# SAP/nested-hashing-psi

Hardware: AMD Instinct MI355X
Metric: server PIE ciphertexts/sec (higher is better)
Workload: dtype u64

## Files before the change

include/piehip.h:

```cpp
#ifndef PIEHIP_H
#define PIEHIP_H

#include <stddef.h>
#include <stdint.h>

#ifdef __cplusplus
extern "C" {
#endif

#define PIEHIP_OK 0
#define PIEHIP_EINVAL (-1)
#define PIEHIP_ESTATE (-2)
#define PIEHIP_EHIP (-3)
#define PIEHIP_ENOMEM (-4)

typedef struct piehip_ctx *piehip_handle;

int piehip_version(void);
const char *piehip_last_error(void);

int piehip_default_moduli(uint32_t N, uint32_t L, uint64_t *q , uint64_t *p );

int piehip_create(piehip_handle *out, uint32_t N, uint32_t L, uint64_t t, const uint64_t *q, const uint64_t *p,
                  int device, void *stream);
// ... 74 lines not shown
int piehip_rccl_attach(piehip_handle h, void *nccl_comm, int nranks, int rank);
int piehip_rccl_destroy(piehip_handle h);
int piehip_rccl_bin_slice(uint32_t b_total, int nranks, int rank, uint32_t *bin_lo, uint32_t *bin_hi);
int piehip_rccl_broadcast(piehip_handle h, int root, void *d_buf, size_t bytes);
int piehip_rccl_broadcast_query(piehip_handle h, int root);
int piehip_gather_results(piehip_handle h, uint32_t b_total, int root, void *d_out);
int piehip_gather_results_host(piehip_handle h, uint32_t b_total, int root, uint64_t **results);
int piehip_rccl_wait(piehip_handle h, uint32_t timeout_ms);
int piehip_rccl_abort(piehip_handle h);
int piehip_rccl_agree(piehip_handle h, int ok, int *all_ok, uint32_t timeout_ms);

int piehip_ntt(piehip_handle h, uint64_t *limbs, uint32_t nlimbs, uint32_t mod_base, uint32_t mod_count, int inverse);
int piehip_eval_add(piehip_handle h, const uint64_t *x, const uint64_t *y, uint64_t *out);
int piehip_eval_mult_plain(piehip_handle h, const uint64_t *x, const uint64_t *pt, uint64_t *out);
int piehip_eval_mult(piehip_handle h, const uint64_t *x, const uint64_t *y, uint32_t nct, int relin, uint64_t *out);
int piehip_eval_automorph(piehip_handle h, const uint64_t *x, uint32_t g, const uint64_t *rk, uint64_t *out);
int piehip_encode(piehip_handle h, const int64_t *slots, uint32_t npt, uint32_t B, uint64_t *out);
int piehip_base_convert(piehip_handle h, int which, const uint64_t *in, uint32_t npoly, uint64_t *out);

int piehip_rotation_galois(piehip_handle h, int32_t index, uint32_t *g);
int piehip_load_rotation_keys(piehip_handle h, uint32_t nkeys, const int32_t *indices, const uint64_t *keys);
int piehip_fhepie_load_table(piehip_handle h, uint32_t npie, uint32_t K, uint32_t b, uint32_t E, const int64_t *slots,
                             const int64_t *masks);
int piehip_fhepie_set_index(piehip_handle h, const uint64_t *idx);
int piehip_fhepie_run(piehip_handle h);
int piehip_fhepie_get_results(piehip_handle h, uint64_t *out);

int piehip_client_keygen(piehip_handle h, uint64_t seed, uint64_t *sk);
int piehip_client_relin_keygen(piehip_handle h, const uint64_t *sk, uint64_t seed, uint64_t *evk);
int piehip_client_rot_keygen(piehip_handle h, const uint64_t *sk, int32_t index, uint64_t seed, uint64_t *rk);
int piehip_client_encrypt(piehip_handle h, const uint64_t *sk, const int64_t *slots, uint32_t nct, uint32_t B,
                          const uint64_t *seeds, uint64_t *out);
int piehip_client_decrypt(piehip_handle h, const uint64_t *sk, const uint64_t *ct, uint32_t nct, uint32_t B, int64_t *slots);

int piehip_expand_uniform(piehip_handle h, const uint8_t *seeds , uint32_t n, uint64_t *out );
int piehip_expand_uniform_device(piehip_handle h, const uint8_t *seeds , uint32_t n, void *d_out );
int piehip_stage_minus_seeded_q(piehip_handle h, uint32_t q, const uint64_t *c0 , const uint8_t *seed );
int piehip_stage_index_row_seeded_q(piehip_handle h, uint32_t q, uint32_t row, const uint64_t *c0 ,
                                    const uint8_t *seeds );
int piehip_stage_index_ct_seeded_q(piehip_handle h, uint32_t q, uint32_t row, uint32_t j, const uint64_t *c0 ,
                                   const uint8_t *seed );
int piehip_run_host_seeded_async(piehip_handle h, const uint64_t *c0idx, const uint8_t *idx_seeds, const uint64_t *c0minus,
                                 const uint8_t *minus_seeds, uint64_t *results);
int piehip_run_host_seeded(piehip_handle h, const uint64_t *c0idx, const uint8_t *idx_seeds, const uint64_t *c0minus,
                           const uint8_t *minus_seeds, uint64_t *results);
int piehip_load_relin_key_seeded(piehip_handle h, const uint64_t *evk0 , const uint8_t *seeds );
int piehip_load_relin_key_seeded_q(piehip_handle h, uint32_t q, const uint64_t *evk0, const uint8_t *seeds);
int piehip_client_encrypt_seeded(piehip_handle h, const uint64_t *sk, const int64_t *slots, uint32_t nct, uint32_t B,
                                 const uint64_t *noise_seeds , const uint8_t *a_seeds ,
                                 uint64_t *c0 );
int piehip_client_relin_keygen_seeded(piehip_handle h, const uint64_t *sk, uint64_t seed, const uint8_t *a_seeds ,
                                      uint64_t *evk0 );

#define PIEHIP_NKERNELS 13
enum {
    PIEHIP_K_STAGE_A = 0,
    PIEHIP_K_NTT_FWD = 1,
    PIEHIP_K_NTT_INV = 2,
    PIEHIP_K_EXPAND = 3,
    PIEHIP_K_TENSOR = 4,
    PIEHIP_K_SCALE = 5,
    PIEHIP_K_DIGITS = 6,
    PIEHIP_K_RELIN = 7,
    PIEHIP_K_MASK = 8,
    PIEHIP_K_ENCODE = 9,
    PIEHIP_K_AUTOMORPH = 10,
    PIEHIP_K_OTHER = 11,
    PIEHIP_K_EVENT_PAIR = 12
};
int piehip_bench_ntt(piehip_handle h, uint32_t nlimbs, uint32_t mod_count, int flags, uint32_t iters, double *ms_per_launch);
int piehip_set_profiling(piehip_handle h, int on);
#define PIEHIP_NKERNELS_V100 12
int piehip_profile_read_n(piehip_handle h, uint32_t n, uint32_t *launches , double *ms , double *alg_bytes );
int piehip_profile_read(piehip_handle h, uint32_t *launches , double *ms , double *alg_bytes );
const char *piehip_kernel_name(int k);

#ifdef __cplusplus
}
#endif
#endif
```

nested_hashing_psi_amd/_lib.py:

```python
import ctypes as C
import os

from .build import LIB_PATH

u64p = C.POINTER(C.c_uint64)
u8p = C.POINTER(C.c_uint8)
i64p = C.POINTER(C.c_int64)
u32p = C.POINTER(C.c_uint32)
i32p = C.POINTER(C.c_int32)
f64p = C.POINTER(C.c_double)

NKERNELS = 13

SYMBOLS = {
    "piehip_version": (C.c_int, []),
    "piehip_last_error": (C.c_char_p, []),
    "piehip_kernel_name": (C.c_char_p, [C.c_int]),
    "piehip_default_moduli": (C.c_int, [C.c_uint32, C.c_uint32, u64p, u64p]),
    "piehip_create": (C.c_int, [C.POINTER(C.c_void_p), C.c_uint32, C.c_uint32, C.c_uint64, u64p, u64p, C.c_int, C.c_void_p]),
    "piehip_destroy": (C.c_int, [C.c_void_p]),
    "piehip_get_moduli": (C.c_int, [C.c_void_p, u64p]),
    "piehip_get_root": (C.c_int, [C.c_void_p, C.c_uint32, u64p]),
    "piehip_get_twiddles": (C.c_int, [C.c_void_p, C.c_uint32, u64p, u64p]),
    "piehip_get_slot_positions": (C.c_int, [C.c_void_p, u32p]),
    "piehip_load_relin_key": (C.c_int, [C.c_void_p, u64p]),
    "piehip_load_db": (C.c_int, [C.c_void_p, C.c_uint32, C.c_uint32, C.c_uint32, u64p, u64p]),
    "piehip_load_db_slots": (C.c_int, [C.c_void_p, C.c_uint32, C.c_uint32, C.c_uint32, C.c_uint32, i64p, i64p]),
    "piehip_build_db": (C.c_int, [C.c_void_p, u64p, C.c_size_t] + [C.c_uint32] * 5 + [C.c_uint64] * 4),
    "piehip_load_db_table": (C.c_int, [C.c_void_p, u64p] + [C.c_uint32] * 5 + [C.c_uint64] * 2),
    "piehip_build_db_bins": (C.c_int, [C.c_void_p, u64p, C.c_size_t] + [C.c_uint32] * 5 + [C.c_uint64] * 4 + [C.c_uint32] * 2),
    "piehip_load_db_table_bins": (C.c_int, [C.c_void_p, u64p] + [C.c_uint32] * 5 + [C.c_uint64] * 2 + [C.c_uint32] * 2),
    "piehip_reserve": (C.c_int, [C.c_void_p, C.c_size_t] + [C.c_uint32] * 7),
    "piehip_get_hash_table": (C.c_int, [C.c_void_p, u64p]),
    "piehip_tabulation_hash": (C.c_int, [C.c_uint64, C.c_uint32, C.c_uint32, u64p, C.c_size_t, u64p]),
    "piehip_client_cuckoo_table": (C.c_int, [C.c_uint64, C.c_uint32, C.c_uint32, C.c_uint32, u64p, C.c_size_t, u64p]),
    "piehip_set_index": (C.c_int, [C.c_void_p, u64p]),
    "piehip_set_minus": (C.c_int, [C.c_void_p, u64p]),
    "piehip_set_index_device": (C.c_int, [C.c_void_p, C.c_void_p]),
    "piehip_set_minus_device": (C.c_int, [C.c_void_p, C.c_void_p]),
    "piehip_run": (C.c_int, [C.c_void_p]),
    "piehip_sync": (C.c_int, [C.c_void_p]),
    "piehip_join": (C.c_int, [C.c_void_p]),
    "piehip_run_into": (C.c_int, [C.c_void_p, C.c_void_p]),
    "piehip_run_host": (C.c_int, [C.c_void_p, u64p, u64p, u64p]),
    "piehip_run_host_async": (C.c_int, [C.c_void_p, u64p, u64p, u64p]),
    "piehip_run_host_wait": (C.c_int, [C.c_void_p]),
    "piehip_stage_minus": (C.c_int, [C.c_void_p, u64p]),
    "piehip_stage_index_row": (C.c_int, [C.c_void_p, C.c_uint32, u64p]),
    "piehip_run_staged": (C.c_int, [C.c_void_p, u64p]),
    "piehip_stage_minus_q": (C.c_int, [C.c_void_p, C.c_uint32, u64p]),
    "piehip_stage_index_row_q": (C.c_int, [C.c_void_p, C.c_uint32, C.c_uint32, u64p]),
    "piehip_stage_index_ct_q": (C.c_int, [C.c_void_p, C.c_uint32, C.c_uint32, C.c_uint32, u64p]),
    "piehip_stage_reset": (C.c_int, [C.c_void_p]),
    "piehip_host_buffers_q": (C.c_int, [C.c_void_p, C.c_uint32, C.POINTER(u64p), C.POINTER(u64p), C.POINTER(u64p)]),
    "piehip_load_relin_key_q": (C.c_int, [C.c_void_p, C.c_uint32, u64p]),
    "piehip_host_buffers": (C.c_int, [C.c_void_p, C.POINTER(u64p), C.POINTER(u64p), C.POINTER(u64p)]),
    "piehip_set_run_streams": (C.c_int, [C.c_void_p, C.c_uint32]),
    "piehip_set_graph": (C.c_int, [C.c_void_p, C.c_int]),
    "piehip_attach_database": (C.c_int, [C.c_void_p, C.c_void_p]),
    "piehip_set_query_batch": (C.c_int, [C.c_void_p, C.c_uint32]),
    "piehip_get_query_batch": (C.c_int, [C.c_void_p, u32p]),
    "piehip_set_index_q": (C.c_int, [C.c_void_p, C.c_uint32, u64p]),
    "piehip_set_minus_q": (C.c_int, [C.c_void_p, C.c_uint32, u64p]),
    "piehip_set_index_device_q": (C.c_int, [C.c_void_p, C.c_uint32, C.c_void_p]),
    "piehip_set_minus_device_q": (C.c_int, [C.c_void_p, C.c_uint32, C.c_void_p]),
# ... 78 lines not shown
```

nested_hashing_psi_amd/csrc/kernels.hpp:

```cpp
#pragma once
#include <hip/hip_runtime.h>

#include <atomic>
#include <vector>

#include "params.hpp"

namespace piehip {

struct PerDeviceOnce {
    std::atomic<unsigned long long> done{0};
    bool first_on_current_device()
    {
        int dev = 0;
        if (hipGetDevice(&dev) != hipSuccess || dev < 0 || dev > 63) return true;
        const unsigned long long bit = 1ULL << dev;
        return (done.fetch_or(bit) & bit) == 0;
    }
};

struct NttPlan {
    const u64 *tables;
    const u64 *twp;
    const u64 *twc;
    const u64 *twc_fold;
    const u64 *twk16 = nullptr;
    const u64 *twk16_fold = nullptr;
    const DevConsts *dc;
    u32 N, logN;
    u32 num_cus;
    u32 max_slots = 0;
    bool force_generic;
    u32 transform_cus() const
    {
        if (!max_slots) return num_cus;
        const u32 c = (max_slots + 1) / 2;
        return c < num_cus ? (c ? c : 1u) : num_cus;
    }
};

void build_twc_table(const u64 *nat_pairs, u32 logN, u32 s0, std::vector<u64> &out);
u32 ntt_fast_s0(u32 logN);
struct NttExtra {
    u64 *copy_out = nullptr;
    u32 copy_K = 1, copy_L = 1, copy_M = 1;
    u32 skip_L = 0, skip_M = 0;
    bool lazy_out = false;
    bool folded = false;
    bool x_lane_in = false;
};
void build_twk16_table(const u64 *nat_pairs, u32 s0, u32 slice_log, std::vector<u64> &out);
void ntt16_sigma_inverse_map(u32 logN, u32 s0, std::vector<u32> &map);
struct Ntt16Digits {
    const u64 *d2;
    size_t stride2;
    u64 *dig;
    u32 nb, L;
};
bool launch_ntt16(const NttPlan &pl, bool folded, u64 *data, u32 nlimbs, u32 mod_base, u32 mod_count, bool inverse, bool sigma,
                  hipStream_t st, const NttExtra *ex, const Ntt16Digits *dg = nullptr);
inline bool ntt16_applies(const NttPlan &pl, bool folded)
{
    return !pl.force_generic && pl.twp && (folded ? (pl.twk16_fold && (pl.logN == 14 || pl.logN == 15)) : (pl.twk16 && pl.logN == 13));
}
bool launch_ntt_fast(const u64 *twp, const u64 *twc, const DevConsts *dc, u32 N, u32 logN, u32 s0, u64 *data, u32 nlimbs, u32 mod_base,
                     u32 mod_count, bool inverse, bool sigma, u32 num_cus, hipStream_t st, const u64 *lift_src = nullptr,
                     u32 lift_L = 0, u32 sigma_split = 0, const NttExtra *ex = nullptr);
bool ntt_supports_extra(const NttPlan &pl, bool folded);
bool launch_ntt_digits(const NttPlan &pl, const u64 *d2, u64 *dig, u32 nb, u32 L, bool sigma, bool folded_layout,
                       hipStream_t st);
void ntt_sigma_inverse_map(u32 logN, u32 s0, std::vector<u32> &map);
void launch_ntt(const NttPlan &pl, u64 *data, u32 nlimbs, u32 mod_base, u32 mod_count, bool inverse, hipStream_t st,
                bool sigma = false, bool folded = false, const NttExtra *ex = nullptr);

struct StageAXOut {
    u64 *out = nullptr;
    u32 M = 0, logns = 0;
};
void launch_stage_a(const DevConsts *dc, u32 N, u32 L, u32 K, u32 b, u32 E, const u64 *idx, const u64 *minus,
                    const u64 *db, u64 *acc, hipStream_t st, bool small_moduli, u32 bstride = 0, u32 h0 = 0, u32 hn = 0, u32 nq = 1,
                    u32 q = 0, const StageAXOut *xo = nullptr);
static const u32 STAGE_A_MAX_QUERIES = 8;
struct StageAQueries {
    const u64 *idx[STAGE_A_MAX_QUERIES];
    const u64 *minus[STAGE_A_MAX_QUERIES];
};
void launch_stage_a_batch(const DevConsts *dc, u32 N, u32 L, u32 K, u32 b, u32 E, const StageAQueries &qs, u32 nq, const u64 *db,
                          u64 *acc, hipStream_t st, bool small_moduli, u32 bstride = 0, u32 h0 = 0, u32 hn = 0,
                          const StageAXOut *xo = nullptr);

void set_small_moduli(bool v);

void launch_expand_q_to_qp(const DevConsts *dc, u32 N, u32 L, const u64 *in, size_t in_stride_outer,
                           size_t in_stride_inner, u32 n_outer, u64 *out, u32 out_polys, u32 out_slot, hipStream_t st,
                           bool fold = false, bool skip_q = false);
void launch_scale_pq_expand(const DevConsts *dc, u32 N, u32 L, const u64 *in, size_t in_stride_outer,
                            size_t in_stride_inner, u32 n_outer, u64 *out, u32 out_polys, u32 out_slot, hipStream_t st,
                            bool fold = false);
void launch_expand_both(const DevConsts *dc, u32 N, u32 L, const u64 *x, size_t sx, const u64 *y, size_t sy, size_t si, u32 n_outer,
                        u64 *out, hipStream_t st, bool fold = false, bool skip_q = false);
void launch_tensor(const DevConsts *dc, u32 N, u32 M, const u64 *e, u64 *d, u32 nb, hipStream_t st);
void launch_scale_round(const DevConsts *dc, u32 N, u32 L, const u64 *d, u32 nb, u64 *out01, size_t stride01, u64 *out2,
                        size_t stride2, hipStream_t st, bool fold = false, bool fold_comp2 = false);
void launch_digits(const DevConsts *dc, u32 N, u32 L, const u64 *d2, size_t stride2, u32 nb, u64 *dig, hipStream_t st,
                   bool fold = false);
void launch_relin_mac(const DevConsts *dc, u32 N, u32 L, const u64 *d01, size_t stride01, const u64 *dig, const u64 *key,
                      const u64 *mask, u64 *out, u32 nb, hipStream_t st, const u32 *out_map = nullptr, size_t key_stride = 0,
                      u32 key_group = 1, u32 sigma_T = 0, u32 sigma_kp = 16, u32 mask_div = 1);
void launch_bcast_mul_plain(const DevConsts *dc, u32 N, u32 L, const u64 *x, size_t xs, u32 group, const u64 *pt, size_t ps_outer,
                            size_t ps_inner, u64 *out, u32 nct, hipStream_t st);
void launch_rot_prepare(const DevConsts *dc, u32 N, u32 L, const u64 *x, const u32 *maps, u32 map_group, bool acc, bool identity_first,
                        u64 *d01, u64 *d2, u32 nct, hipStream_t st);
void launch_sum_mul_plain(const DevConsts *dc, u32 N, u32 L, const u64 *x, u32 group, const u64 *pt, size_t pt_stride, u64 *out,
// ... 37 lines not shown
```

nested_hashing_psi_amd/csrc/kernels_ntt16.hip:

```cpp
#include "kernels.hpp"
#include "ntt16_kernel.h"

namespace piehip {

void build_twk16_table(const u64 *nat_pairs, u32 s0, u32 slice_log, std::vector<u64> &out)
{
    if (slice_log == 14)
        ntt16::build_twk_table_t<14>(nat_pairs, s0, out);
    else
        ntt16::build_twk_table_t<13>(nat_pairs, s0, out);
}

void ntt16_sigma_inverse_map(u32 logN, u32 s0, std::vector<u32> &map)
{
    const u32 N = 1u << logN, n = N >> s0;
    map.resize(N);
    for (u32 p = 0; p < N; p++) map[p] = (p / n) * n + ntt16::lane_to_std_t(p % n, n / 16);
}

template <u32 LOGNS>
static void launch_ntt16_t(const ntt16::Args &a, bool inverse, bool lift, u32 num_cus, hipStream_t st)
{
    typedef ntt16::Geo<LOGNS> G;
    constexpr size_t lds = (size_t)G::LDS_WORDS * sizeof(u64);
    static PerDeviceOnce attr[3];
    if (attr[inverse ? 1 : (lift ? 2 : 0)].first_on_current_device()) {
        if (inverse)
            (void)hipFuncSetAttribute((const void *)ntt16::ntt16_kernel_t<LOGNS, true>, hipFuncAttributeMaxDynamicSharedMemorySize, (int)lds);
        else if (lift)
            (void)hipFuncSetAttribute((const void *)ntt16::ntt16_kernel_t<LOGNS, false, true>, hipFuncAttributeMaxDynamicSharedMemorySize, (int)lds);
        else
            (void)hipFuncSetAttribute((const void *)ntt16::ntt16_kernel_t<LOGNS, false>, hipFuncAttributeMaxDynamicSharedMemorySize, (int)lds);
    }
    const u32 slots = (LOGNS == 13 ? 2u : 1u) * num_cus;
    const u32 grid = a.nitems < slots ? a.nitems : slots;
    if (inverse)
        hipLaunchKernelGGL((ntt16::ntt16_kernel_t<LOGNS, true>), dim3(grid), dim3(G::T), lds, st, a);
    else if (lift)
        hipLaunchKernelGGL((ntt16::ntt16_kernel_t<LOGNS, false, true>), dim3(grid), dim3(G::T), lds, st, a);
    else
        hipLaunchKernelGGL((ntt16::ntt16_kernel_t<LOGNS, false>), dim3(grid), dim3(G::T), lds, st, a);
}

bool launch_ntt16(const NttPlan &pl, bool folded, u64 *data, u32 nlimbs, u32 mod_base, u32 mod_count, bool inverse, bool sigma,
                  hipStream_t st, const NttExtra *ex, const Ntt16Digits *dg)
{
    const u64 *twk = folded ? pl.twk16_fold : pl.twk16;
    const u32 s0 = folded ? 1u : 0u;
    const u32 slice_log = pl.logN - s0;
    if (pl.force_generic || !twk || !pl.twp || (slice_log != 13 && slice_log != 14)) return false;
    if (!inverse && !sigma) return false;
    ntt16::Args a;
    a.data = data;
    a.twp = reinterpret_cast<const ntt16::u64x2 *>(pl.twp);
    a.twk = reinterpret_cast<const ntt16::u64x2 *>(twk);
    a.dc = pl.dc;
    a.N = pl.N;
    a.s0 = s0;
    a.nitems = nlimbs << s0;
    a.mod_base = mod_base;
    a.mod_count = mod_count;
    a.flags = 0;
    if (inverse && !sigma) a.flags |= ntt16::F_STD_IN;
    if (inverse && folded) a.flags |= ntt16::F_FOLDED;
    if (inverse && !sigma && ex && ex->copy_out && ex->x_lane_in) a.flags |= ntt16::F_X_LANE_IN;
    if (!inverse && ex && ex->lazy_out) a.flags |= ntt16::F_LAZY_OUT;
    a.skip_L = (ex && !inverse) ? ex->skip_L : 0;
    a.skip_M = ex ? ex->skip_M : 0;
    a.copy_out = (ex && inverse && !sigma) ? ex->copy_out : nullptr;
    a.copy_K = ex ? ex->copy_K : 1;
    a.copy_L = ex ? ex->copy_L : 1;
    a.copy_M = ex ? ex->copy_M : 1;
    a.lift_first = ~0u;
    a.data2 = nullptr;
    a.lift_src = nullptr;
    a.lift_stride = 0;
    a.lift_L = 1;
    if (dg && !inverse) {
        a.lift_first = a.nitems;
        a.nitems += (dg->nb * dg->L * dg->L) << s0;
        a.data2 = dg->dig;
        a.lift_src = dg->d2;
        a.lift_stride = dg->stride2;
        a.lift_L = dg->L;
    }
    const bool lift = a.lift_first != ~0u;
    if (slice_log == 14)
        launch_ntt16_t<14>(a, inverse, lift, pl.transform_cus(), st);
    else
        launch_ntt16_t<13>(a, inverse, lift, pl.transform_cus(), st);
    return true;
}

}
```

nested_hashing_psi_amd/csrc/ntt16_kernel.h:

```cpp
#pragma once
#include <vector>

#include "madasm.h"
#include "params.hpp"

namespace piehip {
namespace ntt16 {

typedef u64 u64x2 __attribute__((ext_vector_type(2)));

template <u32 LOGNS>
struct Geo {
    static constexpr u32 LOGN = LOGNS;
    static constexpr u32 NS = 1u << LOGNS;
    static constexpr u32 T = NS / 16;
    static constexpr u32 W = T / 64;
    static constexpr u32 R = NS / 1024;
    static constexpr u32 LOGR = LOGNS - 10;
    static constexpr u32 CPT = 16 / R;
    static constexpr u32 LDS_WORDS = NS + NS / 16;
    static constexpr u32 TWK_PER_SLICE = W * 15 * 16 + W * 12 * 64;
};
static constexpr u32 LOGN = Geo<13>::LOGN, NS = Geo<13>::NS, T = Geo<13>::T, LDS_WORDS = Geo<13>::LDS_WORDS,
                     TWK_PER_SLICE = Geo<13>::TWK_PER_SLICE;
// ... 114 lines not shown
    } else {
        *p = x[r];
    }
}
typedef __attribute__((address_space(1))) u64 g_u64;
typedef __attribute__((address_space(1))) u64x2 g_u64x2;
__device__ __forceinline__ u64x2 pair_get_global(const u64 *p) { return *(const g_u64x2 *)p; }
__device__ __forceinline__ void pair_put_global(u64x2 v, u64 *p) { *(g_u64x2 *)p = v; }
template <u32 CPT>
__device__ __forceinline__ void row_put_global(const u64 *x, int r, u64 *p)
{
    if (CPT == 2) {
        u64x2 v;
        v.x = x[2 * r], v.y = x[2 * r + 1];
        pair_put_global(v, p);
    } else {
        *(g_u64 *)p = x[r];
    }
}
template <u32 CPT>
__device__ __forceinline__ void row_get_global(u64 *x, int r, const u64 *p)
{
    if (CPT == 2) {
        const u64x2 v = pair_get_global(p);
        x[2 * r] = v.x, x[2 * r + 1] = v.y;
    } else {
        x[r] = *(const g_u64 *)p;
    }
}

__device__ __forceinline__ void wave_sync()
{
    asm volatile("s_waitcnt lgkmcnt(0)" ::: "memory");
    __builtin_amdgcn_wave_barrier();
}

struct Args {
    u64 *data;
    const u64x2 *twp;
    const u64x2 *twk;
    const DevConsts *dc;
    u32 N;
    u32 s0;
    u32 nitems;
    u32 mod_base, mod_count;
    u32 flags;
    u32 skip_L, skip_M;
    u64 *copy_out;
    u32 copy_K, copy_L, copy_M;
    u64 *data2;
    const u64 *lift_src;
    size_t lift_stride;
    u32 lift_first, lift_L;
};
enum : u32 {
    F_STD_IN = 1,
    F_LAZY_OUT = 2,
    F_FOLDED = 4,
    F_X_LANE_IN = 8,
};

template <u32 LOGNS>
inline void build_twk_table_t(const u64 *nat, u32 s0, std::vector<u64> &out)
{
    typedef Geo<LOGNS> G;
    out.assign((size_t)(1u << s0) * G::TWK_PER_SLICE * 2, 0);
    for (u32 blk = 0; blk < (1u << s0); blk++) {
        u64 *o = &out[(size_t)blk * G::TWK_PER_SLICE * 2];
        auto put = [&](size_t dst, size_t src) {
            o[2 * dst] = nat[2 * src];
            o[2 * dst + 1] = nat[2 * src + 1];
        };
        for (u32 w = 0; w < G::W; w++) {
            for (u32 sc = 0; sc < 4; sc++)
                for (u32 jj = 0; jj < (1u << sc); jj++)
                    for (u32 la = 0; la < 16; la++) {
                        const u32 ml = (16 * G::W) << sc;
                        put(((size_t)w * 15 + ((1u << sc) - 1 + jj)) * 16 + la, ((size_t)ml << s0) + (size_t)blk * ml + (((16 * w + la) << sc) + jj));
                    }
            for (u32 l = 0; l < 64; l++) {
                const u32 m11 = 256 * G::W, m12 = 512 * G::W;
                for (u32 jj = 0; jj < 4; jj++)
                    put(G::W * 15 * 16 + ((size_t)w * 12 + jj) * 64 + l, ((size_t)m11 << s0) + (size_t)blk * m11 + 256 * w + 4 * l + jj);
                for (u32 jj = 0; jj < 8; jj++)
                    put(G::W * 15 * 16 + ((size_t)w * 12 + 4 + jj) * 64 + l, ((size_t)m12 << s0) + (size_t)blk * m12 + 512 * w + 8 * l + jj);
            }
        }
    }
}
inline void build_twk_table(const u64 *nat, u32 s0, std::vector<u64> &out) { build_twk_table_t<13>(nat, s0, out); }
inline u32 lane_to_std_t(u32 p, u32 threads)
{
    const u32 tau = (p >> 1) % threads, j = (p >> 1) / threads;
    return 16 * tau + 2 * j + (p & 1);
}
inline u32 lane_to_std(u32 p) { return lane_to_std_t(p, T); }

#ifndef NTT16_STAMP
#define NTT16_STAMP(i)
#endif

#define NTT16_TWL(ml, i) tw[(((u32)(ml)) << a.s0) + blk * (u32)(ml) + (i)]
#define NTT16_FENCE() __builtin_amdgcn_sched_barrier(0)
#define NTT16_PASS_PRIO(p) __builtin_amdgcn_s_setprio(p)
#ifndef NTT16_PF
#define NTT16_PF 3, 0, 3, 2, 1
#endif
#ifndef NTT16_PI
#define NTT16_PI 3, 3, 2, 0, 1
#endif
#define NTT16_PRIO_PICK_(i, a0, a1, a2, a3, a4) ((i) == 0 ? (a0) : (i) == 1 ? (a1) : (i) == 2 ? (a2) : (i) == 3 ? (a3) : (a4))
#define NTT16_PRIO_PICK(i, ...) NTT16_PRIO_PICK_(i, __VA_ARGS__)
#define NTT16_PRIO_F(i) NTT16_PASS_PRIO(NTT16_PRIO_PICK(i, NTT16_PF))
#define NTT16_PRIO_I(i) NTT16_PASS_PRIO(NTT16_PRIO_PICK(i, NTT16_PI))

#ifndef NTT16_LIFT_XCD
#define NTT16_LIFT_XCD 1
#endif
template <u32 LOGNS, bool INV, bool LIFT = false>
__global__ void __launch_bounds__(Geo<LOGNS>::T, 4) ntt16_kernel_t(Args a)
{
    typedef Geo<LOGNS> G;
    constexpr u32 NS = G::NS, T = G::T, R = G::R, LOGR = G::LOGR, CPT = G::CPT, TWK_PER_SLICE = G::TWK_PER_SLICE;
    extern __shared__ __attribute__((aligned(16))) u64 lds[];
    const u32 tau = threadIdx.x;
    const u32 w = __builtin_amdgcn_readfirstlane(tau >> 6), l = tau & 63;
    const u32 la = l >> 2, lc = l & 3;
    u64 *const p1 = lds + phi(CPT * tau);
    u64 *const p2 = lds + phi(1024 * w + l);
    u64 *const p3 = lds + 1088 * w + 68 * la + lc;
    u64 *const p4 = lds + phi(1024 * w + 16 * l);

    u64 x[16];
    auto limb_of = [&](u32 it) -> u32 {
        u32 lb = it >> a.s0;
        if (!INV && a.skip_L) {
            const u32 P = a.skip_M - a.skip_L, per = 2 * P + 2 * a.skip_M;
            const u32 cb = lb / per, r = lb % per;
            lb = cb * 4 * a.skip_M + (r < 2 * P ? (r / P) * a.skip_M + a.skip_L + r % P : 2 * a.skip_M + (r - 2 * P));
        }
        return lb;
    };
    for (u32 item = blockIdx.x; item < a.nitems; item += gridDim.x) {
        u32 tau_ = tau;
        asm volatile("" : "+v"(tau_));
        const u32 voffb = 16 * tau_;
        const u32 coffb = 8 * CPT * tau_;
        const u32 lab = 4 * (tau_ & 60), lb = 16 * (tau_ & 63);
        const bool lift = LIFT && !INV && item >= a.lift_first;
        u32 item_l = item;
        if (lift) {
            item_l = item - a.lift_first;
#if NTT16_LIFT_XCD
            const u32 G = a.lift_L << a.s0, blk8 = 8 * G, within = item_l % blk8;
            if (item_l - within + blk8 <= a.nitems - a.lift_first) item_l = item_l - within + (within & 7) * G + (within >> 3);
#endif
        }
        const u32 blk = item_l & ((1u << a.s0) - 1);
        const u32 limb = lift ? item_l >> a.s0 : limb_of(item);
        u64 *g = (lift ? a.data2 : a.data) + (((size_t)limb << a.s0) + blk) * NS;
        asm("" : "+s"(g));
        const u32 mod = __builtin_amdgcn_readfirstlane(a.mod_base + limb % a.mod_count);
        const DcS dcs = (DcS)(u64)a.dc;
        const u64 q = dcs->mod[mod].q;
        const u64 q2 = 2 * q, q4 = 4 * q;
        ModC mc;
        mc.nql = (u32)(0 - q), mc.nqh = (u32)((0 - q) >> 32), mc.nq4 = 0 - q4, mc.q4 = q4;
        const TwS tw = (TwS)(u64)(a.twp + ((size_t)mod * 2 + (INV ? 1 : 0)) * a.N);
        const u64x2 *__restrict__ twk = a.twk + (((size_t)mod * 2 + (INV ? 1 : 0)) << a.s0) * TWK_PER_SLICE + (size_t)blk * TWK_PER_SLICE;
        const u64x2 *__restrict__ tw3 = twk + (size_t)w * 15 * 16;
        const u64x2 *__restrict__ tw4 = twk + G::W * 15 * 16 + (size_t)w * 12 * 64;
        u64x2 t7[1], t8[2], t9[4], t10[8], t11[4], t12[8];
#define NTT16_LOAD3(dst, sc)                                                       \
    _Pragma("unroll") for (int j_ = 0; j_ < (1 << (sc)); j_++) dst[j_] = *at_bytes(tw3 + 16 * ((1 << (sc)) - 1 + j_), lab)
#define NTT16_LOAD3H(dst, sc, from)                                                \
    _Pragma("unroll") for (int j_ = (from); j_ < (from) + 4; j_++) dst[j_] = *at_bytes(tw3 + 16 * ((1 << (sc)) - 1 + j_), lab)
#define NTT16_LOAD4(dst, first, n)                                                 \
    _Pragma("unroll") for (int j_ = 0; j_ < (n); j_++) dst[j_] = *at_bytes(tw4 + 64 * ((first) + j_), lb)

        if (!INV) {
            NTT16_STAMP(0);
            NTT16_PRIO_F(0);
            if (lift) {
                const u32 LL = a.lift_L, li = __builtin_amdgcn_readfirstlane((limb / LL) % LL), lj = __builtin_amdgcn_readfirstlane(limb % LL);
                const u64 *src = a.lift_src + (size_t)(limb / (LL * LL)) * a.lift_stride + (size_t)li * a.N;
                const u64 qi = dcs->mod[li].q;
                const u64 nqh1 = 0 - (qi / 2 + 1), dq = q - qi;
                auto lift1 = [&](u64 v) -> u64 {
                    u64 r;
                    asm("v_lshl_add_u64 v[126:127], %[v], 0, %[nqh1]\n\t"
                        "v_ashrrev_i32 v125, 31, v127\n\t"
                        "v_bfi_b32 v126, v125, 0, %[dql]\n\t"
                        "v_bfi_b32 v127, v125, 0, %[dqh]\n\t"
                        "v_lshl_add_u64 %[r], %[v], 0, v[126:127]"
                        : [r] "=v"(r)
                        : [v] "v"(v), [nqh1] "s"(nqh1), [dql] "s"((u32)dq), [dqh] "s"((u32)(dq >> 32))
                        : "v125", "v126", "v127");
                    return r;
                };
                if (a.s0 == 1) {
                    u64x2 fw;
                    fw.x = dcs->fold_w[lj];
                    fw.y = dcs->fold_w_sh[lj] >> 1;
                    const Tw t = make_tw(fw);
                    u64 y[16];
#pragma unroll
                    for (int r = 0; r < (int)R; r++) {
                        row_get_global<CPT>(x, r, at_bytes(src + 1024 * r, coffb));
                        row_get_global<CPT>(y, r, at_bytes(src + NS + 1024 * r, coffb));
                    }
#pragma unroll
                    for (int k = 0; k < 16; k++) {
// ... 74 lines not shown
            for (int mm = 0; mm < 8; mm += 2) {
                const int k0 = bfly_lo(mm, 2), k1 = bfly_lo(mm + 1, 2);
                bfly2<false, false>(x[k0], x[k0 + 2], make_tw(t9[k0 >> 2]), x[k1], x[k1 + 2], make_tw(t9[k1 >> 2]), mc);
            }
            NTT16_LOAD4(t11, 0, 4);
            NTT16_FENCE();
#pragma unroll
            for (int k = 0; k < 16; k += 4)
                bfly2<false, false>(x[k], x[k + 1], make_tw(t10[k >> 1]), x[k + 2], x[k + 3], make_tw(t10[(k >> 1) + 1]), mc);
#pragma unroll
            for (int k = 0; k < 16; k++) p3[4 * k + 2 * (k >> 3)] = x[k];
            NTT16_STAMP(6);
            wave_sync();
            NTT16_PRIO_F(4);
#pragma unroll
            for (int j = 0; j < 8; j++) {
                const u64x2 v = *reinterpret_cast<const u64x2 *>(p4 + 2 * j);
                x[2 * j] = v.x;
                x[2 * j + 1] = v.y;
            }
            NTT16_LOAD4(t12, 4, 4);
            NTT16_FENCE();
#pragma unroll
            for (int g4 = 0; g4 < 4; g4++) {
                const Tw t = make_tw(t11[g4]);
                bfly2<false, false>(x[4 * g4], x[4 * g4 + 2], t, x[4 * g4 + 1], x[4 * g4 + 3], t, mc);
                if (g4 == 1) {
                    NTT16_FENCE();
                    _Pragma("unroll") for (int j_ = 4; j_ < 8; j_++) t12[j_] = *at_bytes(tw4 + 64 * (4 + j_), lb);
                    NTT16_FENCE();
                }
            }
            NTT16_FENCE();
#pragma unroll
            for (int k = 0; k < 16; k += 4)
                bfly2<false, false>(x[k], x[k + 1], make_tw(t12[k >> 1]), x[k + 2], x[k + 3], make_tw(t12[(k >> 1) + 1]), mc);
            NTT16_STAMP(7);
            const bool lazy = (a.flags & F_LAZY_OUT) != 0 && !lift;
            if (!lazy) {
#pragma unroll
                for (int k = 0; k < 16; k++) x[k] = csub_neg(csub_neg(csub_neg(x[k], 0 - q4), 0 - q2), 0 - q);
            }
#pragma unroll
            for (int j = 0; j < 8; j++) {
                u64x2 v;
                v.x = x[2 * j], v.y = x[2 * j + 1];
                pair_put_global(v, at_bytes(g + 2 * T * j, voffb));
            }
            NTT16_STAMP(8);
        } else {
            NTT16_STAMP(0);
            NTT16_PRIO_I(0);
            NTT16_LOAD4(t12, 4, 4);
            const bool is_x = (a.flags & F_STD_IN) && a.copy_out && (limb / (2 * a.copy_L)) % a.copy_K == 0;
            u64 *co = nullptr;
            if (is_x) {
                const u32 bin = limb / (2 * a.copy_L * a.copy_K), cc = (limb / a.copy_L) & 1, i = limb % a.copy_L;
                co = a.copy_out + (((((size_t)bin * 4 + cc) * a.copy_M + i) << a.s0) + blk) * NS;
                asm("" : "+s"(co));
            }
            const bool x_in = is_x && (a.flags & F_X_LANE_IN);
            if ((a.flags & F_STD_IN) && !x_in) {
                u64 yv[16];
                const u64 *gw = g + 1024 * w;
#pragma unroll
                for (int j = 0; j < 8; j++) {
                    const u64x2 v = pair_get_global(at_bytes(gw + 128 * j, lb));
                    yv[2 * j] = v.x, yv[2 * j + 1] = v.y;
                }
                {
                    u64 *const pw = lds + phi(1024 * w + 2 * l);
#pragma unroll
                    for (int j = 0; j < 8; j++) {
                        u64x2 v;
                        v.x = yv[2 * j], v.y = yv[2 * j + 1];
                        *reinterpret_cast<u64x2 *>(pw + 136 * j) = v;
                    }
                }
                wave_sync();
#pragma unroll
                for (int j = 0; j < 8; j++) {
                    const u64x2 v = *reinterpret_cast<const u64x2 *>(p4 + 2 * j);
                    x[2 * j] = v.x;
                    x[2 * j + 1] = v.y;
                }
                if (is_x) {
#pragma unroll
                    for (int j = 0; j < 8; j++) {
                        u64x2 v;
                        v.x = x[2 * j], v.y = x[2 * j + 1];
                        pair_put_global(v, at_bytes(co + 2 * T * j, voffb));
                    }
                }
            } else {
                const u64 *src = x_in ? co : g;
                asm("" : "+s"(src));
#pragma unroll
                for (int j = 0; j < 8; j++) {
                    const u64x2 v = pair_get_global(at_bytes(src + 2 * T * j, voffb));
                    x[2 * j] = v.x, x[2 * j + 1] = v.y;
                }
            }
            NTT16_FENCE();
            _Pragma("unroll") for (int j_ = 4; j_ < 8; j_++) t12[j_] = *at_bytes(tw4 + 64 * (4 + j_), lb);
            NTT16_FENCE();
            NTT16_PRIO_I(1);
#pragma unroll
            for (int k = 0; k < 16; k += 4) {
                bfly2<true, false>(x[k], x[k + 1], make_tw(t12[k >> 1]), x[k + 2], x[k + 3], make_tw(t12[(k >> 1) + 1]), mc);
                if (k == 4) {
                    NTT16_FENCE();
                    NTT16_LOAD4(t11, 0, 4);
                    NTT16_FENCE();
                }
            }
            NTT16_LOAD3(t10, 3);
            NTT16_FENCE();
#pragma unroll
            for (int g4 = 0; g4 < 4; g4++) {
                const Tw t = make_tw(t11[g4]);
                bfly2<true, false>(x[4 * g4], x[4 * g4 + 2], t, x[4 * g4 + 1], x[4 * g4 + 3], t, mc);
            }
            NTT16_STAMP(1);
            NTT16_STAMP(2);
#pragma unroll
            for (int j = 0; j < 8; j++) {
                u64x2 v;
                v.x = x[2 * j];
                v.y = x[2 * j + 1];
                *reinterpret_cast<u64x2 *>(p4 + 2 * j) = v;
            }
            wave_sync();
            NTT16_STAMP(3);
            NTT16_PRIO_I(2);
#pragma unroll
            for (int k = 0; k < 16; k++) x[k] = p3[4 * k + 2 * (k >> 3)];
            NTT16_LOAD3(t9, 2);
            NTT16_FENCE();
#pragma unroll
            for (int k = 0; k < 16; k += 4)
                bfly2<true, false>(x[k], x[k + 1], make_tw(t10[k >> 1]), x[k + 2], x[k + 3], make_tw(t10[(k >> 1) + 1]), mc);
            NTT16_LOAD3(t8, 1);
            NTT16_LOAD3(t7, 0);
            NTT16_FENCE();
#pragma unroll
            for (int mm = 0; mm < 8; mm += 2) {
// ... 78 lines not shown
```

nested_hashing_psi_amd/csrc/piehip.cpp:

```cpp
#include "piehip_ctx.hpp"

#include <random>

using namespace piehip;

static thread_local std::string g_err;
static const char *KNAMES[PIEHIP_NKERNELS] = {"stage_a_mac", "ntt_fwd", "ntt_inv",  "expand",   "tensor",    "scale_round",
                                              "digits",      "relin",   "mask_mul", "encode",   "automorph", "other",
                                              "event_pair"};
static const u32 ENCODE_CHUNK = 256;
static void free_workspace(piehip_ctx *h);

namespace piehip {

int fail(int code, const std::string &msg)
{
    g_err = msg;
    return code;
}

void join_pending(piehip_ctx *h)
{
    if (!h->pending_join) return;
    for (size_t g = 0; g < h->ev_join.size(); g++) (void)hipStreamWaitEvent(h->stream, h->ev_join[g], 0);
    h->pending_join = false;
}

void mark_dirty(piehip_ctx *h) { h->inputs_dirty = true; }

void drop_graph(piehip_ctx *h)
{
    if (h->gexec) (void)hipGraphExecDestroy(h->gexec);
    h->gexec = nullptr;
}

hipEvent_t prof_event(piehip_ctx *h)
{
    if (h->pool_used == h->pool.size()) {
        hipEvent_t e;
        if (hipEventCreate(&e) != hipSuccess) return nullptr;
        h->pool.push_back(e);
    }
    return h->pool[h->pool_used++];
}

int dev_alloc(u64 **p, size_t words)
{
    *p = nullptr;
    if (!words) return PIEHIP_OK;
    hipError_t e = hipMalloc((void **)p, words * sizeof(u64));
    if (e != hipSuccess) return fail(PIEHIP_ENOMEM, std::string("hipMalloc: ") + hipGetErrorString(e));
    return PIEHIP_OK;
}
void dev_free(u64 **p)
{
    if (*p) (void)hipFree(*p);
    *p = nullptr;
}

int ws_alloc(piehip_ctx *h, MulWs &w, u32 nb)
{
    const size_t N = h->hp.N, L = h->hp.L, M = h->hp.M;
// ... 924 lines not shown
```

nested_hashing_psi_amd/csrc/piehip_run.cpp:

```cpp
#include "piehip_ctx.hpp"

using namespace piehip;

namespace piehip {

void ntt(piehip_ctx *h, u64 *data, u32 nlimbs, u32 mod_base, u32 mod_count, bool inv, bool sigma, bool fold, const NttExtra *ex)
{
    ProfScope ps(h, inv ? PIEHIP_K_NTT_INV : PIEHIP_K_NTT_FWD, 16.0 * h->hp.N * nlimbs);
    launch_ntt(h->plan, data, nlimbs, mod_base, mod_count, inv, h->stream, sigma && h->sigma_on, fold && h->fold_on, ex);
}
bool xq_reuse(const piehip_ctx *h) { return h->sigma_on && ntt_supports_extra(h->plan, h->fold_on); }

void enqueue_keyswitch(piehip_ctx *h, MulWs &w, u32 nb, const u64 *key, const u64 *mask, u64 *out, bool sigma, bool fold,
                       size_t key_stride, u32 key_group, bool out_is_result, bool digits_ready)
{
    const u32 N = h->hp.N, L = h->hp.L;
    const size_t LN = h->LN();
    const double W = 8.0 * N;
    set_small_moduli(h->small_moduli);
    bool fused = digits_ready;
    if (!fused && h->sigma_on && h->d_twc && h->hp.logN <= 14 && !(sigma && ntt16_applies(h->plan, fold && h->fold_on))) {
        ProfScope ps(h, PIEHIP_K_NTT_FWD, 16.0 * N * nb * L * L);
        fused = launch_ntt_digits(h->plan, w.d2c, w.dig, nb, L, sigma && h->sigma_on, fold && h->fold_on, h->stream);
    }
    if (!fused) {
        {
            ProfScope ps(h, PIEHIP_K_DIGITS, W * nb * (L + (double)L * L));
            launch_digits(h->d_dc, N, L, w.d2c, LN, nb, w.dig, h->stream, fold && h->fold_on);
        }
        ntt(h, w.dig, nb * L * L, 0, L, false, sigma, fold);
    }
    {
        if (h->wait_before_results && out_is_result) (void)hipStreamWaitEvent(h->stream, h->wait_before_results, 0);
        if (h->chain_armed && out_is_result) {
            h->chain_armed = false;
            (void)hipEventRecord(h->ev_chain, h->stream);
        }
        ProfScope ps(h, PIEHIP_K_RELIN, W * (nb * ((double)L * L + 2 * L + 2 * L + (mask ? L : 0)) + 2.0 * L * L));
        launch_relin_mac(h->d_dc, N, L, w.d01, 2 * LN, w.dig, key, mask, out, nb, h->stream,
                         (sigma && h->sigma_on) ? h->d_sigma_inv : nullptr, key_stride, key_group,
                         (sigma && h->sigma_on) ? h->sigma_T : 0, h->sigma_kp, mask ? h->mask_div : 1);
    }
}

struct RunKey {
    const u64 *key;
    size_t stride;
    u32 group;
};
static RunKey run_key(const piehip_ctx *h)
{
    if (h->key_group > 1) return {h->sigma_on ? h->d_evkq_sigma : h->d_evkq, (size_t)h->hp.L * 2 * h->LN(), h->key_group};
    return {h->sigma_on ? h->d_evk_sigma : h->d_evk, 0, 1};
}

void enqueue_mul(piehip_ctx *h, MulWs &w, const u64 *x, size_t sx, const u64 *y, size_t sy, u32 nb, bool relin,
                 const u64 *mask, u64 *out, bool xq_ready, bool out_is_result)
{
    const u32 N = h->hp.N, L = h->hp.L, M = h->hp.M;
    const size_t LN = h->LN();
    const double W = 8.0 * N;
    set_small_moduli(h->small_moduli);
    {
        ProfScope ps(h, PIEHIP_K_EXPAND, W * nb * (4.0 * L + 4.0 * M));
        launch_expand_both(h->d_dc, N, L, x, sx, y, sy, LN, nb, w.eqp, h->stream, h->fold_on, xq_ready);
    }
    {
        NttExtra ex;
        ex.lazy_out = true;
        if (xq_ready) {
            ex.skip_L = L;
            ex.skip_M = M;
        }
        ntt(h, w.eqp, nb * (xq_ready ? 4 * M - 2 * L : 4 * M), 0, M, false, true, true, &ex);
    }
    {
        ProfScope ps(h, PIEHIP_K_TENSOR, W * nb * 7.0 * M);
        launch_tensor(h->d_dc, N, M, w.eqp, w.dqp, nb, h->stream);
    }
    ntt(h, w.dqp, nb * 3 * M, 0, M, true, true, true);
    if (relin) {
        {
            ProfScope ps(h, PIEHIP_K_SCALE, W * nb * (3.0 * M + 3.0 * L));
            launch_scale_round(h->d_dc, N, L, w.dqp, nb, w.d01, 2 * LN, w.d2c, LN, h->stream, h->fold_on, false);
        }
        bool digits_ready = false;
        {
            NttExtra ex;
            ex.lazy_out = true;
            if (h->sigma_on && h->small_moduli && ntt16_applies(h->plan, h->fold_on)) {
                ProfScope ps(h, PIEHIP_K_NTT_FWD, 16.0 * N * nb * (2.0 * L + (double)L * L));
                Ntt16Digits dg = {w.d2c, LN, w.dig, nb, L};
                digits_ready = launch_ntt16(h->plan, h->fold_on, w.d01, nb * 2 * L, 0, L, false, true, h->stream, &ex, &dg);
            }
            if (!digits_ready) ntt(h, w.d01, nb * 2 * L, 0, L, false, true, true, &ex);
        }
        const RunKey k = run_key(h);
        enqueue_keyswitch(h, w, nb, k.key, mask, out, true, true, k.stride, k.group, out_is_result, digits_ready);
    } else {
        {
            ProfScope ps(h, PIEHIP_K_SCALE, W * nb * (3.0 * M + 3.0 * L));
            launch_scale_round(h->d_dc, N, L, w.dqp, nb, out, 3 * LN, out + 2 * LN, 3 * LN, h->stream, h->fold_on, true);
        }
        ntt(h, out, nb * 3 * L, 0, L, false, false, true);
    }
}

static const u32 MAX_RUN_QUEUES = 2;
u32 run_queue_count(const piehip_ctx *h)
{
    const u32 want = h->run_streams ? h->run_streams : (h->b >= 8 ? 2u : 1u);
    return std::min(want, std::min(MAX_RUN_QUEUES, h->b));
}

int ensure_run_queues(piehip_ctx *h, u32 ng)
{
    while (h->side_streams.size() < ng) {
        hipStream_t s = nullptr;
        hipEvent_t e = nullptr;
        HIPCHK(hipStreamCreateWithFlags(&s, hipStreamNonBlocking));
        h->side_streams.push_back(s);
        HIPCHK(hipEventCreateWithFlags(&e, hipEventDisableTiming));
        h->ev_join.push_back(e);
    }
    return PIEHIP_OK;
}

u32 run_group_size(u32 b, u32 ng, u32 g)
{
    if (ng == 2) {
        const u32 first = (4 * b + 3) / 7;
        return g == 0 ? first : b - first;
    }
// ... 227 lines not shown
```

Before: 69050.

## Fuse tensor product into the inverse NTT16 kernel load stage

Adds a TENSOR variant of the ntt16 kernel that computes the ciphertext tensor product (d0=a0*b0, d1=a0*b1+a1*b0, d2=a1*b1) while loading inputs, instead of running a separate tensor kernel that writes dqp and then an inverse NTT that reads it back. This removes one full write and read of the 3*M-limb intermediate and one kernel launch. It includes hand-written inline assembly for lazy reduction and Barrett-style folding, with XCD-aware item remapping. It falls back to the old path when ntt16 does not apply. The risks are register pressure and correctness of the asm reductions.

```diff
diff --git a/include/piehip.h b/include/piehip.h
--- a/include/piehip.h
+++ b/include/piehip.h
@@ -150,7 +150,7 @@
 int piehip_client_relin_keygen_seeded(piehip_handle h, const uint64_t *sk, uint64_t seed, const uint8_t *a_seeds ,
                                       uint64_t *evk0 );
 
-#define PIEHIP_NKERNELS 13
+#define PIEHIP_NKERNELS 14
 enum {
     PIEHIP_K_STAGE_A = 0,
     PIEHIP_K_NTT_FWD = 1,
@@ -164,7 +164,8 @@
     PIEHIP_K_ENCODE = 9,
     PIEHIP_K_AUTOMORPH = 10,
     PIEHIP_K_OTHER = 11,
-    PIEHIP_K_EVENT_PAIR = 12
+    PIEHIP_K_EVENT_PAIR = 12,
+    PIEHIP_K_TENSOR_NTT_INV = 13
 };
 int piehip_bench_ntt(piehip_handle h, uint32_t nlimbs, uint32_t mod_count, int flags, uint32_t iters, double *ms_per_launch);
 int piehip_set_profiling(piehip_handle h, int on);
diff --git a/nested_hashing_psi_amd/_lib.py b/nested_hashing_psi_amd/_lib.py
--- a/nested_hashing_psi_amd/_lib.py
+++ b/nested_hashing_psi_amd/_lib.py
@@ -10,7 +10,7 @@
 i32p = C.POINTER(C.c_int32)
 f64p = C.POINTER(C.c_double)
 
-NKERNELS = 13
+NKERNELS = 14
 
 SYMBOLS = {
     "piehip_version": (C.c_int, []),
diff --git a/nested_hashing_psi_amd/csrc/kernels.hpp b/nested_hashing_psi_amd/csrc/kernels.hpp
--- a/nested_hashing_psi_amd/csrc/kernels.hpp
+++ b/nested_hashing_psi_amd/csrc/kernels.hpp
@@ -59,6 +59,10 @@
 };
 bool launch_ntt16(const NttPlan &pl, bool folded, u64 *data, u32 nlimbs, u32 mod_base, u32 mod_count, bool inverse, bool sigma,
                   hipStream_t st, const NttExtra *ex, const Ntt16Digits *dg = nullptr);
+#ifndef PIEHIP_FUSE_TENSOR
+#define PIEHIP_FUSE_TENSOR 1
+#endif
+bool launch_ntt16_tensor(const NttPlan &pl, bool folded, const u64 *e, u64 *d, u32 nb, u32 M, hipStream_t st);
 inline bool ntt16_applies(const NttPlan &pl, bool folded)
 {
     return !pl.force_generic && pl.twp && (folded ? (pl.twk16_fold && (pl.logN == 14 || pl.logN == 15)) : (pl.twk16 && pl.logN == 13));
diff --git a/nested_hashing_psi_amd/csrc/kernels_ntt16.hip b/nested_hashing_psi_amd/csrc/kernels_ntt16.hip
--- a/nested_hashing_psi_amd/csrc/kernels_ntt16.hip
+++ b/nested_hashing_psi_amd/csrc/kernels_ntt16.hip
@@ -19,13 +19,15 @@
 }
 
 template <u32 LOGNS>
-static void launch_ntt16_t(const ntt16::Args &a, bool inverse, bool lift, u32 num_cus, hipStream_t st)
+static void launch_ntt16_t(const ntt16::Args &a, bool inverse, bool lift, u32 num_cus, hipStream_t st, bool tensor = false)
 {
     typedef ntt16::Geo<LOGNS> G;
     constexpr size_t lds = (size_t)G::LDS_WORDS * sizeof(u64);
-    static PerDeviceOnce attr[3];
-    if (attr[inverse ? 1 : (lift ? 2 : 0)].first_on_current_device()) {
-        if (inverse)
+    static PerDeviceOnce attr[4];
+    if (attr[tensor ? 3 : inverse ? 1 : (lift ? 2 : 0)].first_on_current_device()) {
+        if (tensor)
+            (void)hipFuncSetAttribute((const void *)ntt16::ntt16_kernel_t<LOGNS, true, false, true>, hipFuncAttributeMaxDynamicSharedMemorySize, (int)lds);
+        else if (inverse)
             (void)hipFuncSetAttribute((const void *)ntt16::ntt16_kernel_t<LOGNS, true>, hipFuncAttributeMaxDynamicSharedMemorySize, (int)lds);
         else if (lift)
             (void)hipFuncSetAttribute((const void *)ntt16::ntt16_kernel_t<LOGNS, false, true>, hipFuncAttributeMaxDynamicSharedMemorySize, (int)lds);
@@ -34,7 +36,9 @@
     }
     const u32 slots = (LOGNS == 13 ? 2u : 1u) * num_cus;
     const u32 grid = a.nitems < slots ? a.nitems : slots;
-    if (inverse)
+    if (tensor)
+        hipLaunchKernelGGL((ntt16::ntt16_kernel_t<LOGNS, true, false, true>), dim3(grid), dim3(G::T), lds, st, a);
+    else if (inverse)
         hipLaunchKernelGGL((ntt16::ntt16_kernel_t<LOGNS, true>), dim3(grid), dim3(G::T), lds, st, a);
     else if (lift)
         hipLaunchKernelGGL((ntt16::ntt16_kernel_t<LOGNS, false, true>), dim3(grid), dim3(G::T), lds, st, a);
@@ -76,6 +80,7 @@
     a.lift_src = nullptr;
     a.lift_stride = 0;
     a.lift_L = 1;
+    a.tsrc = nullptr;
     if (dg && !inverse) {
         a.lift_first = a.nitems;
         a.nitems += (dg->nb * dg->L * dg->L) << s0;
@@ -92,4 +97,36 @@
     return true;
 }
 
+bool launch_ntt16_tensor(const NttPlan &pl, bool folded, const u64 *e, u64 *d, u32 nb, u32 M, hipStream_t st)
+{
+#if PIEHIP_FUSE_TENSOR
+    const u64 *twk = folded ? pl.twk16_fold : pl.twk16;
+    const u32 s0 = folded ? 1u : 0u;
+    const u32 slice_log = pl.logN - s0;
+    if (pl.force_generic || !twk || !pl.twp || (slice_log != 13 && slice_log != 14)) return false;
+    ntt16::Args a = {};
+    a.data = d;
+    a.twp = reinterpret_cast<const ntt16::u64x2 *>(pl.twp);
+    a.twk = reinterpret_cast<const ntt16::u64x2 *>(twk);
+    a.dc = pl.dc;
+    a.N = pl.N;
+    a.s0 = s0;
+    a.nitems = (nb * 3 * M) << s0;
+    a.mod_base = 0;
+    a.mod_count = M;
+    a.flags = folded ? ntt16::F_FOLDED : 0;
+    a.copy_K = a.copy_L = a.copy_M = 1;
+    a.lift_first = ~0u;
+    a.lift_L = 1;
+    a.tsrc = e;
+    if (slice_log == 14)
+        launch_ntt16_t<14>(a, true, false, pl.transform_cus(), st, true);
+    else
+        launch_ntt16_t<13>(a, true, false, pl.transform_cus(), st, true);
+    return true;
+#else
+    return false;
+#endif
 }
+
+}
diff --git a/nested_hashing_psi_amd/csrc/ntt16_kernel.h b/nested_hashing_psi_amd/csrc/ntt16_kernel.h
--- a/nested_hashing_psi_amd/csrc/ntt16_kernel.h
+++ b/nested_hashing_psi_amd/csrc/ntt16_kernel.h
@@ -190,6 +190,7 @@
     const u64 *lift_src;
     size_t lift_stride;
     u32 lift_first, lift_L;
+    const u64 *tsrc;
 };
 enum : u32 {
     F_STD_IN = 1,
@@ -255,7 +256,104 @@
 #ifndef NTT16_LIFT_XCD
 #define NTT16_LIFT_XCD 1
 #endif
-template <u32 LOGNS, bool INV, bool LIFT = false>
+#ifndef NTT16_TENSOR_XCD
+#define NTT16_TENSOR_XCD 1
+#endif
+__device__ __forceinline__ u64 csub2_neg(u64 x, u64 negm4, u64 negm2)
+{
+    u32 lo, hi;
+    asm("v_lshl_add_u64 v[126:127], %[x], 0, %[n4]\n\t"
+        "v_ashrrev_i32 v125, 31, v127\n\t"
+        "v_bfi_b32 v122, v125, %[xl], v126\n\t"
+        "v_bfi_b32 v123, v125, %[xh], v127\n\t"
+        "v_lshl_add_u64 v[126:127], v[122:123], 0, %[n2]\n\t"
+        "v_ashrrev_i32 v125, 31, v127\n\t"
+        "v_bfi_b32 %[lo], v125, v122, v126\n\t"
+        "v_bfi_b32 %[hi], v125, v123, v127"
+        : [lo] "=&v"(lo), [hi] "=&v"(hi)
+        : [x] "v"(x), [xl] "v"((u32)x), [xh] "v"((u32)(x >> 32)), [n4] "s"(negm4), [n2] "s"(negm2)
+        : "v122", "v123", "v125", "v126", "v127");
+    return ((u64)hi << 32) | lo;
+}
+__device__ __forceinline__ u64 colacc123_to_4q(u64 c0, u64 c1, u64 c2, u64 mu, u64 nq)
+{
+    u64 r;
+    asm("v_lshrrev_b64 v[118:119], 30, %[c0]\n\t"
+        "v_lshl_add_u64 v[118:119], v[118:119], 0, %[c1]\n\t"
+        "v_lshrrev_b64 v[120:121], 30, v[118:119]\n\t"
+        "v_lshl_add_u64 v[120:121], v[120:121], 0, %[c2]\n\t"
+        "v_lshlrev_b64 v[122:123], 1, v[120:121]\n\t"
+        "v_bfe_u32 v126, v118, 29, 1\n\t"
+        "v_and_b32 v124, 0x3fffffff, %[c0l]\n\t"
+        "v_bfe_u32 v125, v118, 2, 28\n\t"
+        "v_or_b32 v122, v122, v126\n\t"
+        "v_lshl_or_b32 v124, v118, 30, v124\n\t"
+        "v_lshl_or_b32 v125, v120, 28, v125\n\t"
+        "v_mul_hi_u32 v126, v122, %[mul]\n\t"
+        "v_mov_b32 v127, 0\n\t"
+        "v_mad_u64_u32 v[126:127], vcc, v122, %[muh], v[126:127]\n\t"
+        "v_mad_u64_u32 v[126:127], vcc, v123, %[mul], v[126:127]\n\t"
+        "v_mad_u64_u32 v[118:119], s[96:97], v123, %[muh], 0\n\t"
+        "v_lshrrev_b64 v[126:127], 32, v[126:127]\n\t"
+        "v_addc_co_u32 v127, vcc, 0, v127, vcc\n\t"
+        "v_lshl_add_u64 v[126:127], v[118:119], 0, v[126:127]\n\t"
+        "v_mad_u64_u32 v[118:119], vcc, v126, %[nqh], 0\n\t"
+        "v_mad_u64_u32 v[118:119], vcc, v127, %[nql], v[118:119]\n\t"
+        "v_add_u32 v125, v125, v118\n\t"
+        "v_mad_u64_u32 %[r], vcc, v126, %[nql], v[124:125]"
+        : [r] "=v"(r)
+        : [c0] "v"(c0), [c1] "v"(c1), [c2] "v"(c2), [c0l] "v"((u32)c0), [mul] "s"((u32)mu), [muh] "s"((u32)(mu >> 32)),
+          [nql] "s"((u32)nq), [nqh] "s"((u32)(nq >> 32))
+        : "vcc", "s96", "s97", "v118", "v119", "v120", "v121", "v122", "v123", "v124", "v125", "v126", "v127");
+    return r;
+}
+#ifndef NTT16_TENSOR_DEPTH
+#define NTT16_TENSOR_DEPTH 3
+#endif
+template <u32 T, bool TWO>
+__device__ __forceinline__ void tensor_load(u64 (&x)[16], const u64 *pa, const u64 *pb, const u64 *pc, const u64 *pd, u32 voffb, u64 q,
+                                            u64 mu)
+{
+    constexpr int DEPTH = NTT16_TENSOR_DEPTH;
+    const u64 nq = 0 - q, nq2 = 0 - 2 * q, nq4 = 0 - 4 * q;
+    u64x2 va[8], vb[8], vc[8], vd[8];
+#define NTT16_TLOAD(j)                                                           \
+    do {                                                                         \
+        va[j] = pair_get_global(at_bytes(pa + 2 * T * (j), voffb));              \
+        vb[j] = pair_get_global(at_bytes(pb + 2 * T * (j), voffb));              \
+        if (TWO) {                                                               \
+            vc[j] = pair_get_global(at_bytes(pc + 2 * T * (j), voffb));          \
+            vd[j] = pair_get_global(at_bytes(pd + 2 * T * (j), voffb));          \
+        }                                                                        \
+    } while (0)
+#pragma unroll
+    for (int j = 0; j < DEPTH; j++) NTT16_TLOAD(j);
+#pragma unroll
+    for (int j = 0; j < 8; j++) {
+        NTT16_FENCE();
+#pragma unroll
+        for (int k = 0; k < 2; k++) {
+            const u64 fa = csub2_neg(k ? va[j].y : va[j].x, nq4, nq2);
+            const u64 fb = TWO ? csub2_neg(k ? vb[j].y : vb[j].x, nq4, nq2) : csub_neg(k ? vb[j].y : vb[j].x, nq4);
+            const Split30 sa = split30(fa), sb = split30(fb);
+            ColAcc c;
+            c.c0 = mul_u(sa.lo, sb.lo);
+            c.c1 = mad_u(sa.hi, sb.lo, mul_u(sa.lo, sb.hi));
+            c.c2 = mul_u(sa.hi, sb.hi);
+            if (TWO) {
+                const u64 fc = csub2_neg(k ? vc[j].y : vc[j].x, nq4, nq2);
+                const u64 fd = csub2_neg(k ? vd[j].y : vd[j].x, nq4, nq2);
+                colacc_mac(c, split30(fc), split30(fd));
+            }
+            x[2 * j + k] = colacc123_to_4q(c.c0, c.c1, c.c2, mu, nq);
+        }
+        NTT16_FENCE();
+        if (j + DEPTH < 8) NTT16_TLOAD(j + DEPTH);
+    }
+#undef NTT16_TLOAD
+}
+
+template <u32 LOGNS, bool INV, bool LIFT = false, bool TENSOR = false>
 __global__ void __launch_bounds__(Geo<LOGNS>::T, 4) ntt16_kernel_t(Args a)
 {
     typedef Geo<LOGNS> G;
@@ -294,8 +392,25 @@
             if (item_l - within + blk8 <= a.nitems - a.lift_first) item_l = item_l - within + (within & 7) * G + (within >> 3);
 #endif
         }
-        const u32 blk = item_l & ((1u << a.s0) - 1);
-        const u32 limb = lift ? item_l >> a.s0 : limb_of(item);
+        u32 t_d = 0, t_row = 0, t_blk = 0, t_limb = 0;
+        if (TENSOR) {
+            const u32 M_ = a.mod_count;
+#if NTT16_TENSOR_XCD
+            u32 il = item;
+            const u32 within = il % 24;
+            if (il - within + 24 <= a.nitems) il = il - within + (within & 7) * 3 + (within >> 3);
+            const u32 u = il / 3, lm = u >> a.s0;
+            t_d = il % 3, t_blk = u & ((1u << a.s0) - 1), t_row = lm / M_;
+            t_limb = (t_row * 3 + t_d) * M_ + lm % M_;
+#else
+            t_limb = item >> a.s0, t_blk = item & ((1u << a.s0) - 1);
+            t_row = t_limb / (3 * M_), t_d = (t_limb / M_) % 3;
+#endif
+            t_d = __builtin_amdgcn_readfirstlane(t_d), t_row = __builtin_amdgcn_readfirstlane(t_row);
+            t_blk = __builtin_amdgcn_readfirstlane(t_blk), t_limb = __builtin_amdgcn_readfirstlane(t_limb);
+        }
+        const u32 blk = TENSOR ? t_blk : item_l & ((1u << a.s0) - 1);
+        const u32 limb = TENSOR ? t_limb : lift ? item_l >> a.s0 : limb_of(item);
         u64 *g = (lift ? a.data2 : a.data) + (((size_t)limb << a.s0) + blk) * NS;
         asm("" : "+s"(g));
         const u32 mod = __builtin_amdgcn_readfirstlane(a.mod_base + limb % a.mod_count);
@@ -476,7 +591,7 @@
             NTT16_STAMP(0);
             NTT16_PRIO_I(0);
             NTT16_LOAD4(t12, 4, 4);
-            const bool is_x = (a.flags & F_STD_IN) && a.copy_out && (limb / (2 * a.copy_L)) % a.copy_K == 0;
+            const bool is_x = !TENSOR && (a.flags & F_STD_IN) && a.copy_out && (limb / (2 * a.copy_L)) % a.copy_K == 0;
             u64 *co = nullptr;
             if (is_x) {
                 const u32 bin = limb / (2 * a.copy_L * a.copy_K), cc = (limb / a.copy_L) & 1, i = limb % a.copy_L;
@@ -484,7 +599,7 @@
                 asm("" : "+s"(co));
             }
             const bool x_in = is_x && (a.flags & F_X_LANE_IN);
-            if ((a.flags & F_STD_IN) && !x_in) {
+            if (!TENSOR && (a.flags & F_STD_IN) && !x_in) {
                 u64 yv[16];
                 const u64 *gw = g + 1024 * w;
 #pragma unroll
@@ -516,6 +631,17 @@
                         pair_put_global(v, at_bytes(co + 2 * T * j, voffb));
                     }
                 }
+            } else if (TENSOR) {
+                const u32 M_ = a.mod_count;
+                const size_t ss = ((size_t)M_ << a.s0) * NS;
+                const u64 *e0 = a.tsrc + ((((size_t)t_row * 4 * M_ + limb % M_) << a.s0) + blk) * NS;
+                const u64 *pa = e0 + (t_d == 2 ? ss : 0), *pb = e0 + (t_d == 0 ? 2 : 3) * ss, *pc = e0 + ss, *pd = e0 + 2 * ss;
+                asm("" : "+s"(pa), "+s"(pb), "+s"(pc), "+s"(pd));
+                const u64 mu = (dcs->mod[mod].r1 << 59) | (dcs->mod[mod].r0 >> 5);
+                if (t_d == 1)
+                    tensor_load<T, true>(x, pa, pb, pc, pd, voffb, q, mu);
+                else
+                    tensor_load<T, false>(x, pa, pb, pc, pd, voffb, q, mu);
             } else {
                 const u64 *src = x_in ? co : g;
                 asm("" : "+s"(src));
diff --git a/nested_hashing_psi_amd/csrc/piehip.cpp b/nested_hashing_psi_amd/csrc/piehip.cpp
--- a/nested_hashing_psi_amd/csrc/piehip.cpp
+++ b/nested_hashing_psi_amd/csrc/piehip.cpp
@@ -7,7 +7,7 @@
 static thread_local std::string g_err;
 static const char *KNAMES[PIEHIP_NKERNELS] = {"stage_a_mac", "ntt_fwd", "ntt_inv",  "expand",   "tensor",    "scale_round",
                                               "digits",      "relin",   "mask_mul", "encode",   "automorph", "other",
-                                              "event_pair"};
+                                              "event_pair",  "tensor_ntt_inv"};
 static const u32 ENCODE_CHUNK = 256;
 static void free_workspace(piehip_ctx *h);
 
diff --git a/nested_hashing_psi_amd/csrc/piehip_run.cpp b/nested_hashing_psi_amd/csrc/piehip_run.cpp
--- a/nested_hashing_psi_amd/csrc/piehip_run.cpp
+++ b/nested_hashing_psi_amd/csrc/piehip_run.cpp
@@ -74,11 +74,18 @@
         }
         ntt(h, w.eqp, nb * (xq_ready ? 4 * M - 2 * L : 4 * M), 0, M, false, true, true, &ex);
     }
-    {
-        ProfScope ps(h, PIEHIP_K_TENSOR, W * nb * 7.0 * M);
-        launch_tensor(h->d_dc, N, M, w.eqp, w.dqp, nb, h->stream);
-    }
-    ntt(h, w.dqp, nb * 3 * M, 0, M, true, true, true);
+    bool fused = false;
+    if (PIEHIP_FUSE_TENSOR && h->sigma_on && h->small_moduli && ntt16_applies(h->plan, h->fold_on)) {
+        ProfScope ps(h, PIEHIP_K_TENSOR_NTT_INV, W * nb * 7.0 * M);
+        fused = launch_ntt16_tensor(h->plan, h->fold_on, w.eqp, w.dqp, nb, M, h->stream);
+    }
+    if (!fused) {
+        {
+            ProfScope ps(h, PIEHIP_K_TENSOR, W * nb * 7.0 * M);
+            launch_tensor(h->d_dc, N, M, w.eqp, w.dqp, nb, h->stream);
+        }
+        ntt(h, w.dqp, nb * 3 * M, 0, M, true, true, true);
+    }
     if (relin) {
         {
             ProfScope ps(h, PIEHIP_K_SCALE, W * nb * (3.0 * M + 3.0 * L));
```

After: 72210, median of 6. 4.6% higher.
